# pouryashirazian/FemBrain

Hardware: AMD Instinct MI355X
Metric: FEM steps/sec (assemble+PCG) at 1M tets (higher is better)
Workload: dtype f64 arithmetic / f32 stored matrix

## Files before the change

fembrain_amd/csrc/fem_handle.h:

```cpp
#pragma once
#include "comm.h"
#include "common.h"
#include "fem_kernels.h"
#include "fem_plan.h"
#include "plan_device.h"
#include "renumber.h"
#include "delta.h"
#include "subdivide.h"
#include "surface.h"

namespace fb {

struct PipeKernel;

struct PersistState {
  int pipe_mir_knob = -1;
  int persist_fallbacks = 0;
  int persist_launches = 0;
  int persist_rearms = 0;
  double persist_seconds = 0;
  long long persist_iterations = 0;

  int pipe_lines_nodes = 0;
  double pipe_gather_lines[2] = {0, 0};

  bool persist = false;
  int persist_blocks = 0, persist_waves = 0;
  const PipeKernel* kernel = nullptr;
  int pipe_rows = 1;
  int pipe_wmax = 0;
  int pipe_slots_dealt = 0;
// ... 202 lines not shown
```

fembrain_amd/csrc/fem_persist.hip:

```cpp
#include <cmath>
#include <cstring>

#include "fem_handle.h"
#include "pcg_pipe.hip.h"
#include "pcg_pipe2.hip.h"
#include "pcg_pipe_plan.h"

using namespace fb;

namespace fb {

struct PipeKernel {
  int rows;
  bool c16;
  int wmax, klt;
  bool timing, shard, bj, help, xyz;
  const void* fn;
};

namespace {

#define FB_PIPE1(C16, WMAX, KLT, TIMING, SHARD, BJ, HELP, XYZ) \
  {1, C16, WMAX, KLT, TIMING, SHARD, BJ, HELP, XYZ, (const void*)k_pcg_pipe<float, C16, WMAX, KLT, TIMING, SHARD, BJ, HELP, XYZ>}
#define FB_PIPE2(C16, SHARD, XYZ) {2, C16, 12, kPipe2Klt, false, SHARD, false, false, XYZ, (const void*)k_pcg_pipe2<C16, SHARD, XYZ>}
// ... 32 lines not shown
  k.rearm = std::max(0, env_int("FEMBRAIN_PERSIST_REARM", 32));
  k.timing = getenv("FEMBRAIN_PERSIST_TIMING") ? std::max(1, env_int("FEMBRAIN_PERSIST_TIMING", 1)) : 0;
  k.poll_all = env_int("FEMBRAIN_PERSIST_POLL_ALL", 0) != 0;
  k.sharded = env_int("FEMBRAIN_SHARDED_PERSIST", 0) != 0;
  k.shard_relief = env_int("FEMBRAIN_SHARD_RELIEF", -1);
  k.balance = env_int("FEMBRAIN_PIPE_BALANCE", -1);
  k.small = env_int("FEMBRAIN_PIPE_SMALL", 0) != 0;
  k.klt7 = env_int("FEMBRAIN_PIPE_KLT7", 1) != 0;
  k.helpers = env_int("FEMBRAIN_PIPE_HELPERS", -1);
  k.help_minlen = env_int("FEMBRAIN_PIPE_HELP_MINLEN", 16);
  k.xyz = env_int("FEMBRAIN_PIPE_XYZ", -1);
  k.lds_by_width = env_int("FEMBRAIN_PIPE_LDS_BY_WIDTH", 0) != 0;
  k.lds_cap = getenv("FEMBRAIN_PIPE_LDS_CAP") ? std::max(1, env_int("FEMBRAIN_PIPE_LDS_CAP", 1)) : 0;
  k.plain_stores = env_int("FEMBRAIN_PIPE_PLAIN_STORES", -1);
  k.mirror = env_int("FEMBRAIN_PIPE_MIRROR", 1) != 0;
  k.verbose = getenv("FEMBRAIN_TIMING") != nullptr;
  return k;
}

int resolve_pipe_kernel(fb_fem_s* h, const PersistKnobs& kn) {
  PersistState& ps = h->ps;
  PipeKernel want;
  want.rows = ps.pipe_rows;
  want.shard = ps.shard_persist;
  want.bj = h->prm.pcg_variant == FB_PCG_BLOCK_JACOBI;
  want.help = ps.pipe_tasks.p != nullptr;
  want.xyz = ps.pipe_xyz;
  want.c16 = !want.shard && h->c16 != 0;
  want.timing = ps.persist_timing.p != nullptr && want.rows == 1;
  if (want.bj && want.timing) return fail(FB_EINVAL, "FEMBRAIN_PERSIST_TIMING is built for the Jacobi kernel");
// ... 204 lines not shown
  h->ps.sbox = nullptr;
  h->ps.shard_persist = false;
}

void read_persist_timeout(fb_fem_s* h) {
  const char* t = getenv("FEMBRAIN_PERSIST_TIMEOUT_MS");
  const double ms = t ? atof(t) : (h->plan.n_ranks > 1 ? 2000.0 : 50.0);
  h->ps.persist_timeout_ticks = std::max(1LL, (long long)(ms * 1e5));
}

int setup_persist(fb_fem_s* h) {
  const FemPlan& P = h->plan;
  PersistState& ps = h->ps;
  const PersistKnobs kn = read_persist_knobs();
  if (ps.pipe_mir_knob < 0) ps.pipe_mir_knob = kn.mirror ? 1 : 0;
  ps.pipe_timing_level = kn.timing;
  ps.reset_plan(kn.rearm);
  hipDeviceProp_t prop;
  FB_HIP(hipGetDeviceProperties(&prop, h->prm.device));
  const int nb = std::min(kPipeMaxBlocks, ((h->cu_limit > 0 ? std::min(h->cu_limit, prop.multiProcessorCount) : prop.multiProcessorCount) / 8) * 8);
  int w = nb >= 8 ? ceil_div(ceil_div(P.n_slices, 8), nb / 8) : 0;
  if (P.n_ranks == 1 && !P.slice_off.empty()) {
    w = pipe_deal_by_slots(P.slice_off.data(), P.n_slices, nb, w, kn, &ps.pipe_wg_first_host);
    if (!ps.pipe_wg_first_host.empty()) FB_TRY(ps.pipe_wg_first.upload(ps.pipe_wg_first_host, h->stream));
  }
  read_persist_timeout(h);
  const bool explicit_p = h->prm.pcg_variant == FB_PCG_PERSISTENT;
  const bool shard_opt = P.n_ranks > 1 && kn.sharded;
  if (explicit_p && P.n_ranks > 1 && !shard_opt) return fail(FB_EINVAL, "FB_PCG_PERSISTENT on a sharded handle needs FEMBRAIN_SHARDED_PERSIST=1 (unmeasured on multi-GPU hardware)");
  if (explicit_p && h->f64) return fail(FB_EINVAL, "FB_PCG_PERSISTENT needs FB_MATRIX_F32 storage (part of the matrix is kept in LDS as fp32 words)");
// ... 94 lines not shown
  const PipeKernel& K = *ps.kernel;
  PipeArgs pa;
  pa.post = ps.pipe_post.p; pa.flags = ps.pipe_flags.p; pa.error = ps.pipe_flags.p + ps.persist_blocks + ps.pipe_flag_extra + 4; pa.seqs = ps.pipe_flags.p + ps.persist_blocks + ps.pipe_flag_extra + 8;
  pa.producers = ps.pipe_prod.p; pa.prod_count = ps.pipe_prod_count.p; pa.prod_xcd = ps.pipe_prod_xcd.p; pa.plain_local = ps.pipe_plain_local; pa.xcc = ps.pipe_xcc.p;
  pa.start = start; pa.n_iters = n_iters; pa.eps2 = eps * eps; pa.max_iter = max_iter;
  pa.timeout_ticks = ps.persist_timeout_ticks;
  pa.timing = ps.persist_timing.p;
  pa.planes = ps.pipe_planes.p; pa.n_pad = ps.shard_persist ? (size_t)ceil_div(h->plan.n_local, 64) * 64 : (size_t)h->plan.n_slices * 64;
  pa.pstate = ps.pipe_state.p;
  pa.tasks = ps.pipe_tasks.p; pa.n_help = ps.pipe_n_help;
  pa.wg_first = ps.pipe_wg_first.p;
  pa.mirror = ps.pipe_mir.p; pa.mir_addr = ps.pipe_mir_addr.p; pa.mir_wg = ps.pipe_mir_wg.p; pa.mir_pool = ps.pipe_mir_pool.p;
  const int cwaves = K.rows == 2 ? ceil_div(ps.persist_waves, 2) : ps.persist_waves;
  pa.service = cwaves + ps.pipe_help_waves < ps.pipe_wmax ? 1 : 0;
  pa.prefetch_slots = ps.persist_waves >= 9 ? (K.rows == 2 ? 3 : 4) : 0;
  ShardArgs sa;
  memset(&sa, 0, sizeof sa);
  if (ps.shard_persist) {
    sa.rank = h->plan.rank; sa.n_ranks = h->plan.n_ranks; sa.n_owned = h->plan.n_owned; sa.n_halo = h->plan.n_local - h->plan.n_owned;
    sa.box = ps.sbox; sa.peer_box = ps.sbox_peers.p; sa.peer_seg = ps.sh_peer_seg.p; sa.halo_cap = ps.sbox_halo_cap;
    sa.halo_off = ps.sh_halo_off.p; sa.row_send_off = ps.sh_row_send_off.p; sa.row_send_rank = ps.sh_row_send_rank.p; sa.row_send_pos = ps.sh_row_send_pos.p;
    sa.wg_send_mask = ps.sh_wg_send_mask.p; sa.n_senders = ps.sh_n_senders.p; sa.proxy_wg = ps.sh_proxy_wg.p; sa.n_proxy = ps.sh_n_proxy; sa.wg_duty = ps.sh_wg_duty.p; sa.wg_range = ps.sh_wg_range.p;
    sa.delay_ticks = remote_delay_ticks();
  }
  SellView sv = sell_view(h);
  const float *vals = (const float*)h->vals.p, *dlo = (const float*)h->dlo.p;
  const double* inv = K.bj ? h->invblk.p : h->invdiag.p;
  void* args[] = {&sv, &vals, &dlo, &inv, &b, &h->x.p, &h->r.p, &h->Ad.p, &ps.pipe_z.p, &ps.pipe_s.p, &h->d.p, &h->st.p, &pa, &sa};
  const size_t lds = 160 * 1024;
  const dim3 grid(ps.persist_blocks), block(64 * (cwaves + ps.pipe_help_waves + pa.service));
// ... 192 lines not shown
```

fembrain_amd/csrc/pcg_pipe.hip.h:

```cpp
#pragma once
#include "fem_kernels.h"
#include "pcg_pipe_stream.hip.h"
#include "pcg_pipe_onchip.hip.h"
#include "pcg_pipe_mirror.h"

namespace fb {

constexpr int kPipeMaxWaves = 12;
constexpr int kPipeMaxBlocks = 256;
constexpr int kPipeSyncDoubles = 2 * 16 + 2 * kPipeMaxBlocks + 8;
constexpr int kPipeMaxProducers = 64;
constexpr int pipe_slot_bytes(bool c16) { return c16 ? 9 * 256 + 128 : 10 * 256; }
constexpr int pipe_lds_slots(bool c16) { return c16 ? 65 : 62; }
static_assert(sizeof(double) * kPipeSyncDoubles + (size_t)pipe_lds_slots(false) * pipe_slot_bytes(false) <= 160 * 1024, "LDS budget of k_pcg_pipe");
static_assert(sizeof(double) * kPipeSyncDoubles + (size_t)pipe_lds_slots(true) * pipe_slot_bytes(true) <= 160 * 1024, "LDS budget of k_pcg_pipe<c16>");
static_assert(mir_slot_bytes(true) == pipe_slot_bytes(true) && mir_slot_bytes(false) == pipe_slot_bytes(false) && mir_lds_slots(true) == pipe_lds_slots(true) &&
              mir_lds_slots(false) == pipe_lds_slots(false) && kMirWaves == kPipeMaxWaves, "the LDS window's planner sees the kernel's LDS");
static_assert(pipe_lds_slots(true) * pipe_slot_bytes(true) / 4 < 65536 && pipe_lds_slots(false) * pipe_slot_bytes(false) / 4 < 65536, "16-bit LDS word addresses of the mirror layers");

struct PipeArgs {
  unsigned long long* post;
  unsigned int* flags;
  unsigned int* error;
  unsigned int* seqs;
  const int* producers;
  const int* prod_count;
  const int* prod_xcd;
  int plain_local;
  unsigned int* xcc;
  int prefetch_slots;
  int service;
  int start;
  int n_iters;
  double eps2;
  int max_iter;
  long long timeout_ticks;
  long long* timing;
  double* planes;
  size_t n_pad;
  double* pstate;
  const int* wg_first;
  const int4* tasks;
  int n_help;
// ... 405 lines not shown
    if (rvalid) {
      if (XYZ && through) {
        st_sc1_xyz(pl + 3 * (size_t)row, vin[0], vin[1], vin[2]);
      } else if (through) {
#pragma unroll
        for (int a = 0; a < 3; a++) st_sc1_f64(pl + a * xs + cs * (size_t)row, vin[a]);
      } else {
#pragma unroll
        for (int a = 0; a < 3; a++) pl[a * xs + cs * (size_t)row] = vin[a];
      }
      if constexpr (SHARD) shard_send_row(sa, BL, pub, send_beg, send_end, vin);
    }
  };
  auto product = [&](const double* vin, double* y, bool post_sums, bool late_acquire) {
    double* pl = pa.planes + (size_t)(pub & 1u) * 3 * pa.n_pad;
    asm volatile("s_waitcnt vmcnt(0)" ::: "memory");
    __syncthreads();
    lap(0);
    if (post_sums) sums++;
    if (wv != 0 && live && pa.prefetch_slots > 0 && (mir_a > 0 || own_k1 > k_after)) {
      int so_k = so + (mir_a > 0 ? 0 : k_after);
      asm volatile("" : "+s"(so_k));
      pipe_prefetch_values(min(pa.prefetch_slots, mir_a > 0 ? mir_a : own_k1 - k_after), ((unsigned int)so_k * 9u * 64u + (unsigned int)lane) * (unsigned int)sizeof(float), vals);
    }
    if constexpr (SHARD) {
      if (spare) shard_service_product(sa, BL, pa, pub, pl, nb, lane, send_mask, t_limit, bc, failed);
    }
    if (wv == 0) {
      if (lane == 0) st_sc1_u32(pa.flags + blockIdx.x, pub);
      if (post_sums && lane < 2) {
        double t = 0.0;
        for (int w = 0; w < n_waves; w++) t += wsum[lane * 16 + w];
        const unsigned long long bits = (unsigned long long)__double_as_longlong(t), tag = (unsigned long long)sums << 32;
        unsigned long long* post = pa.post + ((size_t)(sums & 1u) * nb + blockIdx.x) * 4 + 2 * lane;
        st_sc1_u64(post, (bits >> 32) | tag);
// ... 27 lines not shown
      }
      if (failed && lane == 0) st_sc1_u32(pa.error, 1u);
      if (late_acquire) __builtin_amdgcn_fence(__ATOMIC_ACQUIRE, "agent");
      if (plain_cand && !xcc_known && !failed) {
        const bool same = my_prod < 0 || ld_sc1_u32(pa.xcc + my_prod) == ((pub << 4) | my_xcc);
        const bool all_same = __ballot(!same) == 0ULL;
        if (lane == 0) bc[5] = all_same ? 1.0 : 0.0;
      }
      asm volatile("s_waitcnt vmcnt(0)" ::: "memory");
      if (lane == 0) bc[3] = (failed || ld_sc1_u32(pa.error) != 0u) ? 1.0 : 0.0;
    }
    __syncthreads();
    lap(1);
    if (uniform_flag(bc[3] != 0.0 || (SHARD && bc[4] != 0.0))) { failed = true; return; }
    if (plain_cand && !xcc_known) { through = !uniform_flag(bc[5] != 0.0); xcc_known = true; }
    double y0 = 0, y1 = 0, y2 = 0;
    if (rvalid) {
      MT u00 = m00, u01 = m01, u02 = m02, u11 = m11, u12 = m12, u22 = m22;
      asm volatile("" : "+v"(u00), "+v"(u01), "+v"(u02), "+v"(u11), "+v"(u12), "+v"(u22));
      const double l00 = (double)u00, l01 = (double)u01, l02 = (double)u02, l11 = (double)u11, l12 = (double)u12, l22 = (double)u22;
      y0 = l00 * vin[0] + l01 * vin[1] + l02 * vin[2];
      y1 = l01 * vin[0] + l11 * vin[1] + l12 * vin[2];
      y2 = l02 * vin[0] + l12 * vin[1] + l22 * vin[2];
    }
    long long tseam = tprev;
    if (live) {
      if constexpr (kMir) {
        if (mir_a > 0) {
          int so_k = so;
          asm volatile("" : "+s"(so_k));
          pipe_stream_slots<C16, XYZ>(mir_a, ((unsigned int)so_k * 9u * 64u + (unsigned int)lane) * (unsigned int)sizeof(float),
                                      ((unsigned int)so_k * 64u + (unsigned int)lane) * (unsigned int)(C16 ? sizeof(short) : sizeof(int)), vals,
                                      C16 ? (const void*)sv.coldelta : (const void*)sv.colidx, pl, pl + xs, pl + 2 * xs, row, y0, y1, y2);
        }
        seam(5, tseam);
        const char* lbase = (const char*)(lds + kPipeSyncDoubles);
        pipe_onchip_slots<C16>(mir_m, max(KL, 0), (const unsigned int*)(lbase + mir_tab) + lane, (const unsigned short*)(lbase + mir_tab) + lane, lres, lcd, lbase, pl, pl + xs,
                               pl + 2 * xs, row, y0, y1, y2);
      }
      if (sizeof(MT) == 4 && KLT >= 16) {
        double gx[KLT][3];
#pragma unroll
        for (int k = 0; k < KLT; k++) {
          const unsigned int col = k < KL ? lds_col(k) : 0u;
          const double* xp = pl + cs * (size_t)col;
          gx[k][0] = k < KL ? xp[0] : 0.0; gx[k][1] = k < KL ? xp[xs] : 0.0; gx[k][2] = k < KL ? xp[2 * xs] : 0.0;
        }
#pragma unroll
        for (int k = 0; k < KLT; k++) if (k < KL) {
          const unsigned int* lk = lres + (size_t)k * kValWords * 64;
          const double x0 = gx[k][0], x1 = gx[k][1], x2 = gx[k][2];
          y0 += (double)__uint_as_float(lk[0 * 64]) * x0 + (double)__uint_as_float(lk[1 * 64]) * x1 + (double)__uint_as_float(lk[2 * 64]) * x2;
          y1 += (double)__uint_as_float(lk[3 * 64]) * x0 + (double)__uint_as_float(lk[4 * 64]) * x1 + (double)__uint_as_float(lk[5 * 64]) * x2;
// ... 288 lines not shown
```

fembrain_amd/csrc/pcg_pipe_plan.h:

```cpp
#pragma once
#include <algorithm>
#include <cstdio>
#include <cstdlib>
#include <vector>

#include "common.h"
#include "fem_plan.h"
#include "pcg_pipe2.hip.h"

namespace fb {

struct PersistKnobs {
  int pcg_persist = -1;
  int min_waves = 2;
  bool rows2 = false;
  int rearm = 32;
  int timing = 0;
  bool poll_all = false;
  bool sharded = false;
  int shard_relief = -1;
  int balance = -1;
  bool small = false;
  bool klt7 = true;
  int helpers = -1;
  int help_minlen = 16;
  int xyz = -1;
  bool lds_by_width = false;
  int lds_cap = 0;
  int plain_stores = -1;
  bool mirror = true;
  bool verbose = false;
};

inline int pipe_deal_by_slots(const int* slice_off, int n_slices, int nb, int w, const PersistKnobs& kn, std::vector<int>* wg_first) {
  wg_first->clear();
  if (nb < 8 || w < 1 || w > 2 * kPipeMaxWaves) return w;
  const int per = nb / 8, chunk = ceil_div(n_slices, 8), cap = w <= kPipeMaxWaves ? kPipeMaxWaves : 2 * kPipeMaxWaves;
  long long total = 0, worst = 0;
  for (int b = 0; b < nb; b++) {
    int first, count;
    pipe_slices(n_slices, nb, b, &first, &count);
    const long long sl = count > 0 ? slice_off[first + count] - slice_off[first] : 0;
    total += sl;
    worst = std::max(worst, sl);
  }
// ... 232 lines not shown
```

fembrain_amd/csrc/pcg_pipe_stream.hip.h:

```cpp
#pragma once
#include <hip/hip_runtime.h>

namespace fb {

#define FBP_LOADV(r0, r1, r2, r3, r4, r5, r6, r7, r8)                      \
  "global_load_dword " r0 ", %[voff], %[svals]\n\t"                        \
  "global_load_dword " r1 ", %[voff], %[svals] offset:256\n\t"             \
  "global_load_dword " r2 ", %[voff], %[svals] offset:512\n\t"             \
  "global_load_dword " r3 ", %[voff], %[svals] offset:768\n\t"             \
  "global_load_dword " r4 ", %[voff], %[svals] offset:1024\n\t"            \
  "global_load_dword " r5 ", %[voff], %[svals] offset:1280\n\t"            \
  "global_load_dword " r6 ", %[voff], %[svals] offset:1536\n\t"            \
  "global_load_dword " r7 ", %[voff], %[svals] offset:1792\n\t"            \
  "global_load_dword " r8 ", %[voff], %[svals] offset:2048\n\t"            \
  "v_add_u32_e32 %[voff], 0x900, %[voff]\n\t"
#define FBP_LOADV_A FBP_LOADV("v136", "v137", "v138", "v139", "v140", "v141", "v142", "v143", "v144")
#define FBP_LOADV_B FBP_LOADV("v145", "v146", "v147", "v148", "v149", "v150", "v151", "v152", "v153")
#define FBP_LOADC16(c) "global_load_sshort " c ", %[coff], %[scols]\n\t" "v_add_u32_e32 %[coff], 0x80, %[coff]\n\t"
#define FBP_LOADC32(c) "global_load_dword " c ", %[coff], %[scols]\n\t" "v_add_u32_e32 %[coff], 0x100, %[coff]\n\t"
#define FBP_GOFF16(c) "v_add_u32_e32 v122, %[row], " c "\n\t" "v_lshlrev_b32_e32 v122, 3, v122\n\t"
#define FBP_GOFF32(c) "v_lshlrev_b32_e32 v122, 3, " c "\n\t"
#define FBP_GOFF16X(c) "v_add_u32_e32 v122, %[row], " c "\n\t" "v_mul_u32_u24_e32 v122, 24, v122\n\t"
#define FBP_GOFF32X(c) "v_mul_u32_u24_e32 v122, 24, " c "\n\t"
#define FBP_GATHER(g0, g1, g2)                                             \
// ... 22 lines not shown
  FBP_ROW("%[y1]", "v139", "v140", "v141", "v[124:125]", "v[126:127]", "v[128:129]")           \
  FBP_ROW("%[y2]", "v142", "v143", "v144", "v[124:125]", "v[126:127]", "v[128:129]")
#define FBP_COMPUTE_B                                                                          \
  FBP_ROW("%[y0]", "v145", "v146", "v147", "v[130:131]", "v[132:133]", "v[134:135]")           \
  FBP_ROW("%[y1]", "v148", "v149", "v150", "v[130:131]", "v[132:133]", "v[134:135]")           \
  FBP_ROW("%[y2]", "v151", "v152", "v153", "v[130:131]", "v[132:133]", "v[134:135]")
#define FBP_FULL(LOADC, GOFF, cX, cY, LOADV_Y, GATHER_Y, COMPUTE_X, W1, W2) \
  LOADC(cX) LOADV_Y "s_waitcnt vmcnt(" W1 ")\n\t" GOFF(cY) GATHER_Y "s_waitcnt vmcnt(" W2 ")\n\t" COMPUTE_X
#define FBP_PENULT(GOFF, cY, LOADV_Y, GATHER_Y, COMPUTE_X, W3, W4)         \
  LOADV_Y "s_waitcnt vmcnt(" W3 ")\n\t" GOFF(cY) GATHER_Y "s_waitcnt vmcnt(" W4 ")\n\t" COMPUTE_X
#define FBP_LAST(COMPUTE_X) "s_waitcnt vmcnt(0)\n\t" COMPUTE_X
#define FBP_BODY(LOADC, GOFF) FBP_BODYG(LOADC, GOFF, FBP_GATHER_A, FBP_GATHER_B, "22", "13", "21", "12")
#define FBP_BODYG(LOADC, GOFF, GATHER_A, GATHER_B, W1, W2, W3, W4)                                                                                 \
           \
  "s_nop 4\n\t"                                                                                                 \
                         \
  LOADC("v154")                                                                                                 \
  "s_cmp_lt_i32 %[n], 2\n\t"                                                                                    \
  "s_cbranch_scc1 .Lfbp_one_%=\n\t"                                                                             \
  LOADC("v155")                                                                                                 \
  FBP_LOADV_A                                                                                                   \
  "s_waitcnt vmcnt(10)\n\t"                                                                                     \
  "s_branch .Lfbp_g0_%=\n"                                                                                      \
  ".Lfbp_one_%=:\n\t"                                                                                           \
  FBP_LOADV_A                                                                                                   \
  "s_waitcnt vmcnt(9)\n"                                                                                        \
  ".Lfbp_g0_%=:\n\t"                                                                                            \
  GOFF("v154") GATHER_A                                                                                     \
                                                                                 \
  ".Lfbp_even_%=:\n\t"                                                                                          \
  "s_cmp_lt_i32 %[n], 3\n\t"                                                                                    \
  "s_cbranch_scc1 .Lfbp_even_tail_%=\n\t"                                                                       \
  FBP_FULL(LOADC, GOFF, "v154", "v155", FBP_LOADV_B, GATHER_B, FBP_COMPUTE_A, W1, W2)                               \
  "s_sub_i32 %[n], %[n], 1\n\t"                                                                                 \
                                                                                  \
  "s_cmp_lt_i32 %[n], 3\n\t"                                                                                    \
  "s_cbranch_scc1 .Lfbp_odd_tail_%=\n\t"                                                                        \
  FBP_FULL(LOADC, GOFF, "v155", "v154", FBP_LOADV_A, GATHER_A, FBP_COMPUTE_B, W1, W2)                               \
  "s_sub_i32 %[n], %[n], 1\n\t"                                                                                 \
  "s_branch .Lfbp_even_%=\n"                                                                                    \
  ".Lfbp_even_tail_%=:\n\t"                                                                                     \
  "s_cmp_lt_i32 %[n], 2\n\t"                                                                                    \
  "s_cbranch_scc1 .Lfbp_even_last_%=\n\t"                                                                       \
  FBP_PENULT(GOFF, "v155", FBP_LOADV_B, GATHER_B, FBP_COMPUTE_A, W3, W4)                                            \
  FBP_LAST(FBP_COMPUTE_B)                                                                                       \
  "s_branch .Lfbp_end_%=\n"                                                                                     \
  ".Lfbp_even_last_%=:\n\t"                                                                                     \
  FBP_LAST(FBP_COMPUTE_A)                                                                                       \
  "s_branch .Lfbp_end_%=\n"                                                                                     \
  ".Lfbp_odd_tail_%=:\n\t"                                                                                      \
  "s_cmp_lt_i32 %[n], 2\n\t"                                                                                    \
  "s_cbranch_scc1 .Lfbp_odd_last_%=\n\t"                                                                        \
  FBP_PENULT(GOFF, "v154", FBP_LOADV_A, GATHER_A, FBP_COMPUTE_B, W3, W4)                                            \
  FBP_LAST(FBP_COMPUTE_A)                                                                                       \
  "s_branch .Lfbp_end_%=\n"                                                                                     \
  ".Lfbp_odd_last_%=:\n\t"                                                                                      \
  FBP_LAST(FBP_COMPUTE_B)                                                                                       \
  ".Lfbp_end_%=:\n\t"
#define FBP_CLOBBERS                                                                                                                   \
  "memory", "scc", "v120", "v121", "v122", "v123", "v124", "v125", "v126", "v127", "v128", "v129", "v130", "v131", "v132", "v133",      \
  "v134", "v135", "v136", "v137", "v138", "v139", "v140", "v141", "v142", "v143", "v144", "v145", "v146", "v147", "v148", "v149",      \
  "v150", "v151", "v152", "v153", "v154", "v155"

__device__ __forceinline__ void pipe_prefetch_values(int n, unsigned int voff, const float* vals);

template <typename T>
__device__ __forceinline__ T* scalar_ptr(T* p) {
  const unsigned long long b = (unsigned long long)p;
  const unsigned int lo = __builtin_amdgcn_readfirstlane((unsigned int)b), hi = __builtin_amdgcn_readfirstlane((unsigned int)(b >> 32));
  return (T*)(((unsigned long long)hi << 32) | lo);
}

__device__ __forceinline__ void pipe_prefetch_values(int n, unsigned int voff, const float* vals) {
  vals = scalar_ptr(vals);
  n = __builtin_amdgcn_readfirstlane(n);
  asm volatile("s_nop 4\n\t"
               "s_cmp_lt_i32 %[n], 1\n\t"
// ... 32 lines not shown
                 : [svals] "s"(vals), [scols] "s"(cols), [spl0] "s"(pl0), [spl1] "s"(pl1), [spl2] "s"(pl2), [row] "v"(row)
                 : FBP_CLOBBERS);
  } else if (C16) {
    asm volatile(FBP_BODY(FBP_LOADC16, FBP_GOFF16)
                 : [y0] "+v"(y0), [y1] "+v"(y1), [y2] "+v"(y2), [voff] "+v"(voff), [coff] "+v"(coff), [n] "+s"(n)
                 : [svals] "s"(vals), [scols] "s"(cols), [spl0] "s"(pl0), [spl1] "s"(pl1), [spl2] "s"(pl2), [row] "v"(row)
                 : FBP_CLOBBERS);
  } else {
    asm volatile(FBP_BODY(FBP_LOADC32, FBP_GOFF32)
                 : [y0] "+v"(y0), [y1] "+v"(y1), [y2] "+v"(y2), [voff] "+v"(voff), [coff] "+v"(coff), [n] "+s"(n)
                 : [svals] "s"(vals), [scols] "s"(cols), [spl0] "s"(pl0), [spl1] "s"(pl1), [spl2] "s"(pl2), [row] "v"(row)
                 : FBP_CLOBBERS);
  }
}

}
```

fembrain_amd/csrc/plan_api.cpp:

```cpp
#include <cstring>
#include <string>
#include <vector>

#include "../../include/fembrain_hip.h"
#include "../../include/fembrain_hip_testing.h"
#include "fem_plan.h"
#include "renumber.h"
#include "pcg_pipe_mirror.h"

namespace fb {
int fail(int code, const char* fmt, ...);
}

struct fb_plan_s {
  fb::FemPlan plan;
};

extern "C" {

int fb_plan_create(fb_plan_t* out, int n_nodes, int n_tets, const int* tets, int n_fixed_dofs, const int* fixed_dofs, int n_ranks,
                   int rank, const int* node_splits) {
  if (!out) return fb::fail(FB_EINVAL, "null output");
  fb_plan_s* p = new fb_plan_s;
  int rc = fb::build_fem_plan(p->plan, n_nodes, n_tets, tets, n_fixed_dofs, fixed_dofs, n_ranks, rank, node_splits);
  if (rc != FB_OK) {
    delete p;
    return rc;
  }
  *out = p;
  return FB_OK;
}
// ... 48 lines not shown
  if (rc != FB_OK) return rc;
  memcpy(old_of_new, o.data(), sizeof(int) * (size_t)n_nodes);
  return FB_OK;
}

int fb_plan_shard_vote(int n_nodes, int n_tets, const int* tets, int n_ranks, int rank, const int* node_splits, int out[3]) {
  if (!tets || !out) return fb::fail(FB_EINVAL, "null argument");
  unsigned long long sum = 0;
  int splits_sum = 0;
  fb::shard_neighbour_count(n_nodes, n_tets, tets, n_ranks, rank, node_splits, &out[0], &sum, &splits_sum, &out[1], &out[2]);
  return FB_OK;
}

int fb_plan_mirror_model(fb_plan_t p, int nb, int c16, int klt, int out[4]) {
  if (!p || !out || nb < 8 || (nb & 7) || (klt != 6 && klt != 7)) return fb::fail(FB_EINVAL, "bad argument");
  const fb::FemPlan& P = p->plan;
  const int* so = P.slice_off.data();
  const int* ci = P.colidx.data();
  out[0] = out[1] = out[3] = 0;
  out[2] = 1 << 30;
  for (int b = 0; b < nb; b++) {
    const int xcd = b & 7, j = b >> 3, per = nb >> 3, chunk = (P.n_slices + 7) >> 3, lo_s = xcd * chunk;
    int len = P.n_slices - lo_s;
    len = len < 0 ? 0 : (len > chunk ? chunk : len);
    const int base = len / per, rem = len - base * per;
    const int first = lo_s + j * base + (j < rem ? j : rem);
    const int count = std::min(base + (j < rem ? 1 : 0), fb::kMirWaves);
    if (count <= 0) continue;
    const int lo = first * 64, hi = std::min((first + count) * 64, P.n_owned);
    fb::MirWave mw[fb::kMirWaves];
    for (int w = 0; w < count; w++) {
      const int sl = first + w, width = so[sl + 1] - so[sl];
      int hist[256] = {0};
      for (int l = 0; l < 64; l++) {
        const int dk = fb::mir_lane_diag(so, ci, sl, l, P.n_owned);
        if (dk >= 0 && dk < 256) hist[dk]++;
      }
      int d = -1, best = 0;
      for (int k = 0; k < width && k < 256; k++)
        if (hist[k] > best) { best = hist[k]; d = k; }
      int m = 0;
      if (d >= 0)
        for (; m < fb::kMirMax && d - 1 - m >= 0; m++) {
          int n = 0;
          for (int l = 0; l < 64; l++) n += fb::mir_lane_lower(so, ci, sl, d - 1 - m, l, lo, hi) ? 1 : 0;
          if (n < fb::kMirLanes) break;
        }
      mw[w].d = d; mw[w].m = m; mw[w].width = width;
    }
    auto misses = [&]() {
      int e = 0;
      for (int w = 0; w < count; w++)
        for (int k = 0; k < mw[w].m; k++)
          for (int l = 0; l < 64; l++) e += fb::mir_lane_addr(so, ci, first, mw, w, k, l, lo, hi, c16 != 0) < 0 ? 1 : 0;
      return e;
    };
    bool ok = fb::mir_wg_layout(mw, count, klt, c16 != 0, 0, false);
    int E = ok ? misses() : 0;
    ok = ok && E <= fb::kMirPoolMax && fb::mir_wg_layout(mw, count, klt, c16 != 0, E, true);
    if (ok) { E = misses(); ok = fb::mir_wg_gains(mw, count, klt, c16 != 0); }
    if (!ok) { fb::mir_wg_plain(mw, count, klt, c16 != 0); E = 0; }
    for (int w = 0; w < count; w++) { out[0] += mw[w].m; out[2] = std::min(out[2], mw[w].p); }
    out[1] += E;
    out[3] += ok ? 1 : 0;
  }
  return FB_OK;
}

}
```

fembrain_amd/lib.py:

```python
import ctypes as C
import os
import subprocess

import numpy as np

_HERE = os.path.dirname(os.path.abspath(__file__))
LIB_PATH = os.path.join(_HERE, "libfembrain_hip.so")

FB_OK, FB_EINVAL, FB_EDEVICE, FB_ENOMEM, FB_ESOLVER, FB_ECOMM = 0, -1, -2, -3, -4, -5
FB_MATRIX_F32, FB_MATRIX_F64, FB_MATRIX_AUTO = 0, 1, 2
FB_XCH_COLLECTIVE, FB_XCH_P2P, FB_XCH_P2P_SUMS, FB_XCH_P2P_FUSED = 1, 2, 3, 4
FB_PCG_MERGED, FB_PCG_REFERENCE, FB_PCG_PERSISTENT, FB_PCG_BLOCK_JACOBI = 0, 1, 3, 4
FB_PCG_PATH_TWO_LAUNCH, FB_PCG_PATH_PERSISTENT, FB_PCG_PATH_FALLBACK, FB_PCG_PATH_RESOLVED = 0, 1, 2, 3
FB_SPMV_AUTO, FB_SPMV_ROWS, FB_SPMV_SPLIT = 0, 1, 2
FB_INTEGRATOR_VOLUME_CONSERVING, FB_INTEGRATOR_NEWMARK = 0, 1
FB_RENUMBER_AUTO, FB_RENUMBER_ON, FB_RENUMBER_OFF = 0, 1, -1
FB_RESYNC_FULL, FB_RESYNC_DELTA_MERGED, FB_RESYNC_DELTA_REBUILT = 0, 1, 2
FB_CUT_BAKE, FB_CUT_CARRY = 0, 1
FB_CUT_NOTHING, FB_CUT_DONE, FB_CUT_UNHANDLED, FB_CUT_DRY = 0, 1, 2, 3
FB_CUT_UNHANDLED_IDS = 64

_dp = C.POINTER(C.c_double)
_fp = C.POINTER(C.c_float)
_ip = C.POINTER(C.c_int)
# ... 137 lines not shown
        "fb_comm_info": (C.c_int, [vp, _ip, _ip, _ip]),
        "fb_comm_create_local": (C.c_int, [C.POINTER(vp), C.c_int, C.c_int, C.c_char_p, C.c_size_t, C.c_int]),
        "fb_comm_test_allgather": (C.c_int, [vp, C.c_void_p, C.c_void_p, C.c_size_t]),
        "fb_fem_create_from_poly": (C.c_int, [C.POINTER(vp), vp, C.c_int, _ip, C.POINTER(FemParams)]),
        "fb_fem_device_plan_get": (C.c_longlong, [vp, C.c_char_p, _ip, C.c_longlong]),
        "fb_fem_plan_on_device": (C.c_int, [vp]),
        "fb_fem_assembly_kernel": (C.c_int, [vp]),
        "fb_fem_assembly_wide_slices": (C.c_int, [vp]),
        "fb_plan_create": (C.c_int, [C.POINTER(vp), C.c_int, C.c_int, _ip, C.c_int, _ip, C.c_int, C.c_int, _ip]),
        "fb_plan_destroy": (C.c_int, [vp]),
        "fb_plan_slab_order": (C.c_int, [C.c_int, _dp, C.c_int, _ip, _ip, _ip, _ip]),
        "fb_plan_shard_vote": (C.c_int, [C.c_int, C.c_int, _ip, C.c_int, C.c_int, _ip, _ip]),
        "fb_plan_info": (C.c_int, [vp, _ip]),
        "fb_plan_get": (C.c_int, [vp, C.c_char_p, _ip, C.c_size_t]),
        "fb_plan_mirror_model": (C.c_int, [vp, C.c_int, C.c_int, C.c_int, _ip]),
    }
    poly_sig = {
        "fb_fem_transport": (C.c_int, [vp]),
        "fb_fem_set_exchange_mode": (C.c_int, [vp, C.c_int]),
        "fb_fem_persist_rearms": (C.c_int, [vp]),
        "fb_fem_persist_helpers": (C.c_int, [vp]),
        "fb_fem_persist_gather": (C.c_int, [vp, C.POINTER(C.c_double), C.POINTER(C.c_double)]),
        "fb_fem_persist_mirror": (C.c_int, [vp, _ip, _ip, _ip]),
        "fb_fem_renumbering": (C.c_int, [vp, _ip, _ip]),
        "fb_fem_owned_nodes": (C.c_int, [vp, _ip]),
        "fb_fem_halo_info": (C.c_int, [vp, _ip, _ip]),
        "fb_fem_sharded_persist": (C.c_int, [vp]),
        "fb_fem_set_sharded_persist": (C.c_int, [vp, C.c_int]),
        "fb_fem_time_exchange": (C.c_int, [vp, C.c_int, _dp, _dp]),
        "fb_fem_time_element_stiffness": (C.c_int, [vp, C.c_int, _dp]),
# ... 84 lines not shown
```

include/fembrain_hip_testing.h:

```cpp
#ifndef FEMBRAIN_HIP_TESTING_H
#define FEMBRAIN_HIP_TESTING_H
#include <stddef.h>
#ifdef __cplusplus
extern "C" {
#endif

typedef struct fb_plan_s* fb_plan_t;

int fb_plan_create(fb_plan_t* out, int n_nodes, int n_tets, const int* tets, int n_fixed_dofs, const int* fixed_dofs,
                   int n_ranks, int rank, const int* node_splits);
int fb_plan_destroy(fb_plan_t p);
int fb_plan_info(fb_plan_t p, int info[12]);
int fb_plan_get(fb_plan_t p, const char* name, int* out, size_t capacity);

int fb_plan_mirror_model(fb_plan_t p, int nb, int c16, int klt, int out[4]);

int fb_plan_slab_order(int n_nodes, const double* xyz, int n_tets, const int* tets, int* old_of_new, int* span_caller, int* span_internal);

int fb_plan_shard_vote(int n_nodes, int n_tets, const int* tets, int n_ranks, int rank, const int* node_splits, int out[3]);

struct fb_comm_s;
int fb_comm_create_local(struct fb_comm_s** out, int rank, int n_ranks, const char* shm_name, size_t outbox_bytes, int device);
int fb_comm_test_allgather(struct fb_comm_s* c, const void* mine, void* all, size_t bytes);

int fb_poly_compile_info(int n_ops, const float* ops16, int n_prims, const float* prims20, int* n_steps, int* n_slots);

#ifdef __cplusplus
}
#endif
#endif
```

Before: 67.74.

## Add opt-in held-slot preload for mirrored PCG pipe SpMV streaming

Adds a FEMBRAIN_PIPE_HOLD knob, off by default, that preloads the first one or two mirrored matrix slots into registers before the barrier. The streamed SpMV then starts from those held values instead of reloading them. It also moves the diagonal-block product ahead of the barrier, passes the on-chip slot pointers differently, and factors the mirror model into a helper exposed through a new window-model query. The goal is to hide global-memory latency at the start of each product, at the cost of more vector registers and more complex inline assembly.

Measured after the change: 66.45. 0.981x the previous value.

```diff
diff --git a/fembrain_amd/csrc/fem_handle.h b/fembrain_amd/csrc/fem_handle.h
--- a/fembrain_amd/csrc/fem_handle.h
+++ b/fembrain_amd/csrc/fem_handle.h
@@ -15,6 +15,7 @@
 
 struct PersistState {
   int pipe_mir_knob = -1;
+  int pipe_hold_knob = -1;
   int persist_fallbacks = 0;
   int persist_launches = 0;
   int persist_rearms = 0;
diff --git a/fembrain_amd/csrc/fem_persist.hip b/fembrain_amd/csrc/fem_persist.hip
--- a/fembrain_amd/csrc/fem_persist.hip
+++ b/fembrain_amd/csrc/fem_persist.hip
@@ -70,6 +70,7 @@
   k.lds_cap = getenv("FEMBRAIN_PIPE_LDS_CAP") ? std::max(1, env_int("FEMBRAIN_PIPE_LDS_CAP", 1)) : 0;
   k.plain_stores = env_int("FEMBRAIN_PIPE_PLAIN_STORES", -1);
   k.mirror = env_int("FEMBRAIN_PIPE_MIRROR", 1) != 0;
+  k.hold = env_int("FEMBRAIN_PIPE_HOLD", 0) != 0;
   k.verbose = getenv("FEMBRAIN_TIMING") != nullptr;
   return k;
 }
@@ -304,6 +305,7 @@
   PersistState& ps = h->ps;
   const PersistKnobs kn = read_persist_knobs();
   if (ps.pipe_mir_knob < 0) ps.pipe_mir_knob = kn.mirror ? 1 : 0;
+  if (ps.pipe_hold_knob < 0) ps.pipe_hold_knob = kn.hold ? 1 : 0;
   ps.pipe_timing_level = kn.timing;
   ps.reset_plan(kn.rearm);
   hipDeviceProp_t prop;
@@ -428,6 +430,7 @@
   const int cwaves = K.rows == 2 ? ceil_div(ps.persist_waves, 2) : ps.persist_waves;
   pa.service = cwaves + ps.pipe_help_waves < ps.pipe_wmax ? 1 : 0;
   pa.prefetch_slots = ps.persist_waves >= 9 ? (K.rows == 2 ? 3 : 4) : 0;
+  pa.hold = ps.pipe_hold_knob != 0 ? 1 : 0;
   ShardArgs sa;
   memset(&sa, 0, sizeof sa);
   if (ps.shard_persist) {
diff --git a/fembrain_amd/csrc/pcg_pipe.hip.h b/fembrain_amd/csrc/pcg_pipe.hip.h
--- a/fembrain_amd/csrc/pcg_pipe.hip.h
+++ b/fembrain_amd/csrc/pcg_pipe.hip.h
@@ -27,6 +27,7 @@
   const int* prod_count;
   const int* prod_xcd;
   int plain_local;
+  int hold;
   unsigned int* xcc;
   int prefetch_slots;
   int service;
@@ -462,11 +463,33 @@
   };
   auto product = [&](const double* vin, double* y, bool post_sums, bool late_acquire) {
     double* pl = pa.planes + (size_t)(pub & 1u) * 3 * pa.n_pad;
+    double y0 = 0, y1 = 0, y2 = 0;
+    auto diag_low = [&]() {
+      if (rvalid) {
+        MT u00 = m00, u01 = m01, u02 = m02, u11 = m11, u12 = m12, u22 = m22;
+        asm volatile("" : "+v"(u00), "+v"(u01), "+v"(u02), "+v"(u11), "+v"(u12), "+v"(u22));
+        const double l00 = (double)u00, l01 = (double)u01, l02 = (double)u02, l11 = (double)u11, l12 = (double)u12, l22 = (double)u22;
+        y0 = l00 * vin[0] + l01 * vin[1] + l02 * vin[2];
+        y1 = l01 * vin[0] + l11 * vin[1] + l12 * vin[2];
+        y2 = l02 * vin[0] + l12 * vin[1] + l22 * vin[2];
+      }
+    };
+    if constexpr (kMir) diag_low();
     asm volatile("s_waitcnt vmcnt(0)" ::: "memory");
     __syncthreads();
     lap(0);
     if (post_sums) sums++;
-    if (wv != 0 && live && pa.prefetch_slots > 0 && (mir_a > 0 || own_k1 > k_after)) {
+    PipeHeld hs;
+    int held = 0;
+    if constexpr (kMir) {
+      held = __builtin_amdgcn_readfirstlane(wv != 0 && live && pa.hold != 0 ? min(mir_a, 2) : 0);
+      int so_k = so;
+      asm volatile("" : "+s"(so_k));
+      pipe_hold_preload<C16>(held, min(pa.prefetch_slots, mir_a) - held, ((unsigned int)so_k * 9u * 64u + (unsigned int)lane) * (unsigned int)sizeof(float),
+                             ((unsigned int)so_k * 64u + (unsigned int)lane) * (unsigned int)(C16 ? sizeof(short) : sizeof(int)), vals,
+                             C16 ? (const void*)sv.coldelta : (const void*)sv.colidx, hs);
+    }
+    if (wv != 0 && live && held == 0 && pa.prefetch_slots > 0 && (mir_a > 0 || own_k1 > k_after)) {
       int so_k = so + (mir_a > 0 ? 0 : k_after);
       asm volatile("" : "+s"(so_k));
       pipe_prefetch_values(min(pa.prefetch_slots, mir_a > 0 ? mir_a : own_k1 - k_after), ((unsigned int)so_k * 9u * 64u + (unsigned int)lane) * (unsigned int)sizeof(float), vals);
@@ -524,29 +547,23 @@
     lap(1);
     if (uniform_flag(bc[3] != 0.0 || (SHARD && bc[4] != 0.0))) { failed = true; return; }
     if (plain_cand && !xcc_known) { through = !uniform_flag(bc[5] != 0.0); xcc_known = true; }
-    double y0 = 0, y1 = 0, y2 = 0;
-    if (rvalid) {
-      MT u00 = m00, u01 = m01, u02 = m02, u11 = m11, u12 = m12, u22 = m22;
-      asm volatile("" : "+v"(u00), "+v"(u01), "+v"(u02), "+v"(u11), "+v"(u12), "+v"(u22));
-      const double l00 = (double)u00, l01 = (double)u01, l02 = (double)u02, l11 = (double)u11, l12 = (double)u12, l22 = (double)u22;
-      y0 = l00 * vin[0] + l01 * vin[1] + l02 * vin[2];
-      y1 = l01 * vin[0] + l11 * vin[1] + l12 * vin[2];
-      y2 = l02 * vin[0] + l12 * vin[1] + l22 * vin[2];
-    }
+    if constexpr (!kMir) diag_low();
     long long tseam = tprev;
     if (live) {
       if constexpr (kMir) {
         if (mir_a > 0) {
-          int so_k = so;
+          int so_k = so + held;
           asm volatile("" : "+s"(so_k));
-          pipe_stream_slots<C16, XYZ>(mir_a, ((unsigned int)so_k * 9u * 64u + (unsigned int)lane) * (unsigned int)sizeof(float),
-                                      ((unsigned int)so_k * 64u + (unsigned int)lane) * (unsigned int)(C16 ? sizeof(short) : sizeof(int)), vals,
-                                      C16 ? (const void*)sv.coldelta : (const void*)sv.colidx, pl, pl + xs, pl + 2 * xs, row, y0, y1, y2);
+          pipe_stream_held<C16>(mir_a, held, ((unsigned int)so_k * 9u * 64u + (unsigned int)lane) * (unsigned int)sizeof(float),
+                                ((unsigned int)so_k * 64u + (unsigned int)lane) * (unsigned int)(C16 ? sizeof(short) : sizeof(int)), vals,
+                                C16 ? (const void*)sv.coldelta : (const void*)sv.colidx, pl, pl + xs, pl + 2 * xs, row, hs, y0, y1, y2);
         }
         seam(5, tseam);
         const char* lbase = (const char*)(lds + kPipeSyncDoubles);
-        pipe_onchip_slots<C16>(mir_m, max(KL, 0), (const unsigned int*)(lbase + mir_tab) + lane, (const unsigned short*)(lbase + mir_tab) + lane, lres, lcd, lbase, pl, pl + xs,
-                               pl + 2 * xs, row, y0, y1, y2);
+        int lane_o = lane;
+        asm volatile("" : "+v"(lane_o));
+        pipe_onchip_slots<C16>(mir_m, max(KL, 0), (const unsigned int*)(lbase + mir_tab) + lane_o, (const unsigned short*)(lbase + mir_tab) + lane_o,
+                               (const unsigned int*)lwave + lane_o, (const short*)(lwave + (size_t)klt_w * 9 * 256) + lane_o, lbase, pl, pl + xs, pl + 2 * xs, row, y0, y1, y2);
       }
       if (sizeof(MT) == 4 && KLT >= 16) {
         double gx[KLT][3];
diff --git a/fembrain_amd/csrc/pcg_pipe_plan.h b/fembrain_amd/csrc/pcg_pipe_plan.h
--- a/fembrain_amd/csrc/pcg_pipe_plan.h
+++ b/fembrain_amd/csrc/pcg_pipe_plan.h
@@ -29,6 +29,7 @@
   int lds_cap = 0;
   int plain_stores = -1;
   bool mirror = true;
+  bool hold = false;
   bool verbose = false;
 };
 
diff --git a/fembrain_amd/csrc/pcg_pipe_stream.hip.h b/fembrain_amd/csrc/pcg_pipe_stream.hip.h
--- a/fembrain_amd/csrc/pcg_pipe_stream.hip.h
+++ b/fembrain_amd/csrc/pcg_pipe_stream.hip.h
@@ -60,53 +60,112 @@
 #define FBP_BODYG(LOADC, GOFF, GATHER_A, GATHER_B, W1, W2, W3, W4)                                                                                 \
            \
   "s_nop 4\n\t"                                                                                                 \
-                         \
-  LOADC("v154")                                                                                                 \
+  FBP_PROLOGUE(LOADC, GOFF, "v154", "v155", FBP_LOADV_A, GATHER_A)                                              \
+  FBP_STEADY(LOADC, GOFF, "v154", "v155", FBP_LOADV_A, FBP_LOADV_B, GATHER_A, GATHER_B, FBP_COMPUTE_A, FBP_COMPUTE_B, W1, W2, W3, W4)
+#define FBP_PROLOGUE(LOADC, GOFF, cA, cB, LOADV_A, GATHER_A)                                                    \
+  LOADC(cA)                                                                                                     \
   "s_cmp_lt_i32 %[n], 2\n\t"                                                                                    \
   "s_cbranch_scc1 .Lfbp_one_%=\n\t"                                                                             \
-  LOADC("v155")                                                                                                 \
-  FBP_LOADV_A                                                                                                   \
+  LOADC(cB)                                                                                                     \
+  LOADV_A                                                                                                       \
   "s_waitcnt vmcnt(10)\n\t"                                                                                     \
   "s_branch .Lfbp_g0_%=\n"                                                                                      \
   ".Lfbp_one_%=:\n\t"                                                                                           \
-  FBP_LOADV_A                                                                                                   \
+  LOADV_A                                                                                                       \
   "s_waitcnt vmcnt(9)\n"                                                                                        \
   ".Lfbp_g0_%=:\n\t"                                                                                            \
-  GOFF("v154") GATHER_A                                                                                     \
+  GOFF(cA) GATHER_A
+#define FBP_STEADY(LOADC, GOFF, cA, cB, LOADV_A, LOADV_B, GATHER_A, GATHER_B, COMPUTE_A, COMPUTE_B, W1, W2, W3, W4) \
                                                                                  \
   ".Lfbp_even_%=:\n\t"                                                                                          \
   "s_cmp_lt_i32 %[n], 3\n\t"                                                                                    \
   "s_cbranch_scc1 .Lfbp_even_tail_%=\n\t"                                                                       \
-  FBP_FULL(LOADC, GOFF, "v154", "v155", FBP_LOADV_B, GATHER_B, FBP_COMPUTE_A, W1, W2)                               \
+  FBP_FULL(LOADC, GOFF, cA, cB, LOADV_B, GATHER_B, COMPUTE_A, W1, W2)                                           \
   "s_sub_i32 %[n], %[n], 1\n\t"                                                                                 \
                                                                                   \
   "s_cmp_lt_i32 %[n], 3\n\t"                                                                                    \
   "s_cbranch_scc1 .Lfbp_odd_tail_%=\n\t"                                                                        \
-  FBP_FULL(LOADC, GOFF, "v155", "v154", FBP_LOADV_A, GATHER_A, FBP_COMPUTE_B, W1, W2)                               \
+  FBP_FULL(LOADC, GOFF, cB, cA, LOADV_A, GATHER_A, COMPUTE_B, W1, W2)                                           \
   "s_sub_i32 %[n], %[n], 1\n\t"                                                                                 \
   "s_branch .Lfbp_even_%=\n"                                                                                    \
   ".Lfbp_even_tail_%=:\n\t"                                                                                     \
   "s_cmp_lt_i32 %[n], 2\n\t"                                                                                    \
   "s_cbranch_scc1 .Lfbp_even_last_%=\n\t"                                                                       \
-  FBP_PENULT(GOFF, "v155", FBP_LOADV_B, GATHER_B, FBP_COMPUTE_A, W3, W4)                                            \
-  FBP_LAST(FBP_COMPUTE_B)                                                                                       \
+  FBP_PENULT(GOFF, cB, LOADV_B, GATHER_B, COMPUTE_A, W3, W4)                                                    \
+  FBP_LAST(COMPUTE_B)                                                                                           \
   "s_branch .Lfbp_end_%=\n"                                                                                     \
   ".Lfbp_even_last_%=:\n\t"                                                                                     \
-  FBP_LAST(FBP_COMPUTE_A)                                                                                       \
+  FBP_LAST(COMPUTE_A)                                                                                           \
   "s_branch .Lfbp_end_%=\n"                                                                                     \
   ".Lfbp_odd_tail_%=:\n\t"                                                                                      \
   "s_cmp_lt_i32 %[n], 2\n\t"                                                                                    \
   "s_cbranch_scc1 .Lfbp_odd_last_%=\n\t"                                                                        \
-  FBP_PENULT(GOFF, "v154", FBP_LOADV_A, GATHER_A, FBP_COMPUTE_B, W3, W4)                                            \
-  FBP_LAST(FBP_COMPUTE_A)                                                                                       \
+  FBP_PENULT(GOFF, cA, LOADV_A, GATHER_A, COMPUTE_B, W3, W4)                                                    \
+  FBP_LAST(COMPUTE_A)                                                                                           \
   "s_branch .Lfbp_end_%=\n"                                                                                     \
   ".Lfbp_odd_last_%=:\n\t"                                                                                      \
-  FBP_LAST(FBP_COMPUTE_B)                                                                                       \
+  FBP_LAST(COMPUTE_B)                                                                                           \
   ".Lfbp_end_%=:\n\t"
+#define FBP_HV_A "%[a0]", "%[a1]", "%[a2]", "%[a3]", "%[a4]", "%[a5]", "%[a6]", "%[a7]", "%[a8]"
+#define FBP_HV_B "%[b0]", "%[b1]", "%[b2]", "%[b3]", "%[b4]", "%[b5]", "%[b6]", "%[b7]", "%[b8]"
+#define FBP_EXPAND(M, ...) M(__VA_ARGS__)
+#define FBP_LOADV_HA FBP_EXPAND(FBP_LOADV, FBP_HV_A)
+#define FBP_LOADV_HB FBP_EXPAND(FBP_LOADV, FBP_HV_B)
+#define FBP_COMPUTE_HA                                                                         \
+  FBP_ROW("%[y0]", "%[a0]", "%[a1]", "%[a2]", "v[124:125]", "v[126:127]", "v[128:129]")        \
+  FBP_ROW("%[y1]", "%[a3]", "%[a4]", "%[a5]", "v[124:125]", "v[126:127]", "v[128:129]")        \
+  FBP_ROW("%[y2]", "%[a6]", "%[a7]", "%[a8]", "v[124:125]", "v[126:127]", "v[128:129]")
+#define FBP_COMPUTE_HB                                                                         \
+  FBP_ROW("%[y0]", "%[b0]", "%[b1]", "%[b2]", "v[130:131]", "v[132:133]", "v[134:135]")        \
+  FBP_ROW("%[y1]", "%[b3]", "%[b4]", "%[b5]", "v[130:131]", "v[132:133]", "v[134:135]")        \
+  FBP_ROW("%[y2]", "%[b6]", "%[b7]", "%[b8]", "v[130:131]", "v[132:133]", "v[134:135]")
+#define FBP_BODYH(LOADC, GOFF)                                                                                  \
+  "s_nop 4\n\t"                                                                                                 \
+  "s_cmp_lt_i32 %[held], 1\n\t"                                                                                 \
+  "s_cbranch_scc1 .Lfbp_h0_%=\n\t"                                                                              \
+  GOFF("%[ca]") FBP_GATHER_A                                                                                    \
+  "s_cmp_lt_i32 %[held], 2\n\t"                                                                                 \
+  "s_cbranch_scc1 .Lfbp_even_last_%=\n\t"                                         \
+  GOFF("%[cb]") FBP_GATHER_B                                                                                    \
+  "s_cmp_lt_i32 %[n], 3\n\t"                                                                                    \
+  "s_cbranch_scc1 .Lfbp_hw3_%=\n\t"                                                                             \
+  LOADC("%[ca]")                                                                                                \
+  "s_cmp_lt_i32 %[n], 4\n\t"                                                                                    \
+  "s_cbranch_scc1 .Lfbp_hw4_%=\n\t"                                                                             \
+  LOADC("%[cb]")                                                                                                \
+  "s_waitcnt vmcnt(5)\n\t"                                   \
+  "s_branch .Lfbp_hc0_%=\n"                                                                                     \
+  ".Lfbp_hw4_%=:\n\t"                                                                                           \
+  "s_waitcnt vmcnt(4)\n\t"                                                                                      \
+  "s_branch .Lfbp_hc0_%=\n"                                                                                     \
+  ".Lfbp_hw3_%=:\n\t"                                                                                           \
+  "s_waitcnt vmcnt(3)\n"                                                                                        \
+  ".Lfbp_hc0_%=:\n\t"                                                                                           \
+  FBP_COMPUTE_HA                                                                                                \
+  "s_cmp_lt_i32 %[n], 3\n\t"                                                                                    \
+  "s_cbranch_scc1 .Lfbp_odd_last_%=\n\t"                                \
+  FBP_LOADV_HA                                                                                                  \
+  "s_cmp_lt_i32 %[n], 4\n\t"                                                                                    \
+  "s_cbranch_scc1 .Lfbp_hw9_%=\n\t"                                                                             \
+  "s_waitcnt vmcnt(10)\n\t"                               \
+  "s_branch .Lfbp_hg2_%=\n"                                                                                     \
+  ".Lfbp_hw9_%=:\n\t"                                                                                           \
+  "s_waitcnt vmcnt(9)\n"                                                                                        \
+  ".Lfbp_hg2_%=:\n\t"                                                                                           \
+  GOFF("%[ca]") FBP_GATHER_A                                                                                    \
+  FBP_COMPUTE_HB                                                                                                \
+  "s_sub_i32 %[n], %[n], 2\n\t"                                                                                 \
+  "s_branch .Lfbp_even_%=\n"                                                                                    \
+  ".Lfbp_h0_%=:\n\t"                                                                                            \
+  FBP_PROLOGUE(LOADC, GOFF, "%[ca]", "%[cb]", FBP_LOADV_HA, FBP_GATHER_A)                                       \
+  FBP_STEADY(LOADC, GOFF, "%[ca]", "%[cb]", FBP_LOADV_HA, FBP_LOADV_HB, FBP_GATHER_A, FBP_GATHER_B, FBP_COMPUTE_HA, FBP_COMPUTE_HB, "22", "13", "21", "12")
 #define FBP_CLOBBERS                                                                                                                   \
   "memory", "scc", "v120", "v121", "v122", "v123", "v124", "v125", "v126", "v127", "v128", "v129", "v130", "v131", "v132", "v133",      \
   "v134", "v135", "v136", "v137", "v138", "v139", "v140", "v141", "v142", "v143", "v144", "v145", "v146", "v147", "v148", "v149",      \
   "v150", "v151", "v152", "v153", "v154", "v155"
+#define FBP_CLOBBERS_HELD                                                                                                              \
+  "memory", "scc", "v120", "v121", "v122", "v123", "v124", "v125", "v126", "v127", "v128", "v129", "v130", "v131", "v132", "v133",      \
+  "v134", "v135"
 
 __device__ __forceinline__ void pipe_prefetch_values(int n, unsigned int voff, const float* vals);
 
@@ -169,4 +228,59 @@
   }
 }
 
-}
+struct PipeHeld {
+  float a[9], b[9];
+  int ca, cb;
+};
+
+template <bool C16>
+__device__ __forceinline__ void pipe_hold_preload(int held, int more, unsigned int voff, unsigned int coff, const float* vals, const void* cols, PipeHeld& h) {
+  vals = scalar_ptr(vals); cols = scalar_ptr(cols);
+  held = __builtin_amdgcn_readfirstlane(held); more = __builtin_amdgcn_readfirstlane(more);
+#define FBP_PRELOAD(LOADC)                                                                                                     \
+  asm volatile("s_nop 4\n\t"                                                                                                   \
+               "s_cmp_lt_i32 %[held], 1\n\t"                                                                                   \
+               "s_cbranch_scc1 .Lfbp_hp_end_%=\n\t"                                                                            \
+               LOADC("%[ca]") FBP_LOADV_HA                                                                                     \
+               "s_cmp_lt_i32 %[held], 2\n\t"                                                                                   \
+               "s_cbranch_scc1 .Lfbp_hp_wait_%=\n\t"   \
+               LOADC("%[cb]") FBP_LOADV_HB                                                                                     \
+               "s_cmp_lt_i32 %[more], 1\n\t"                                                                                   \
+               "s_cbranch_scc1 .Lfbp_hp_wait_%=\n\t"                                                                           \
+               FBP_LOADV("v120", "v121", "v122", "v123", "v124", "v125", "v126", "v127", "v128")                               \
+               "s_cmp_lt_i32 %[more], 2\n\t"                                                                                   \
+               "s_cbranch_scc1 .Lfbp_hp_wait_%=\n\t"                                                                           \
+               FBP_LOADV("v120", "v121", "v122", "v123", "v124", "v125", "v126", "v127", "v128")                               \
+               ".Lfbp_hp_wait_%=:\n\t"                                                                                         \
+               "s_waitcnt vmcnt(0)\n"                                                                                          \
+               ".Lfbp_hp_end_%=:\n\t"                                                                                          \
+               : [a0] "=&v"(h.a[0]), [a1] "=&v"(h.a[1]), [a2] "=&v"(h.a[2]), [a3] "=&v"(h.a[3]), [a4] "=&v"(h.a[4]), [a5] "=&v"(h.a[5]),     \
+                 [a6] "=&v"(h.a[6]), [a7] "=&v"(h.a[7]), [a8] "=&v"(h.a[8]), [b0] "=&v"(h.b[0]), [b1] "=&v"(h.b[1]), [b2] "=&v"(h.b[2]),     \
+                 [b3] "=&v"(h.b[3]), [b4] "=&v"(h.b[4]), [b5] "=&v"(h.b[5]), [b6] "=&v"(h.b[6]), [b7] "=&v"(h.b[7]), [b8] "=&v"(h.b[8]),     \
+                 [ca] "=&v"(h.ca), [cb] "=&v"(h.cb), [voff] "+v"(voff), [coff] "+v"(coff)                                        \
+               : [held] "s"(held), [more] "s"(more), [svals] "s"(vals), [scols] "s"(cols)                                     \
+               : FBP_CLOBBERS_HELD)
+  if (C16) FBP_PRELOAD(FBP_LOADC16);
+  else FBP_PRELOAD(FBP_LOADC32);
+#undef FBP_PRELOAD
+}
+
+template <bool C16>
+__device__ __forceinline__ void pipe_stream_held(int n, int held, unsigned int voff, unsigned int coff, const float* vals, const void* cols, const double* pl0,
+                                                 const double* pl1, const double* pl2, int row, PipeHeld& h, double& y0, double& y1, double& y2) {
+  vals = scalar_ptr(vals); cols = scalar_ptr(cols); pl0 = scalar_ptr(pl0); pl1 = scalar_ptr(pl1); pl2 = scalar_ptr(pl2);
+  n = __builtin_amdgcn_readfirstlane(n); held = __builtin_amdgcn_readfirstlane(held);
+#define FBP_HELD_OPERANDS                                                                                                      \
+               : [y0] "+v"(y0), [y1] "+v"(y1), [y2] "+v"(y2), [voff] "+v"(voff), [coff] "+v"(coff), [n] "+s"(n),               \
+                 [a0] "+v"(h.a[0]), [a1] "+v"(h.a[1]), [a2] "+v"(h.a[2]), [a3] "+v"(h.a[3]), [a4] "+v"(h.a[4]), [a5] "+v"(h.a[5]),     \
+                 [a6] "+v"(h.a[6]), [a7] "+v"(h.a[7]), [a8] "+v"(h.a[8]), [b0] "+v"(h.b[0]), [b1] "+v"(h.b[1]), [b2] "+v"(h.b[2]),     \
+                 [b3] "+v"(h.b[3]), [b4] "+v"(h.b[4]), [b5] "+v"(h.b[5]), [b6] "+v"(h.b[6]), [b7] "+v"(h.b[7]), [b8] "+v"(h.b[8]),     \
+                 [ca] "+v"(h.ca), [cb] "+v"(h.cb)                                                                              \
+               : [held] "s"(held), [svals] "s"(vals), [scols] "s"(cols), [spl0] "s"(pl0), [spl1] "s"(pl1), [spl2] "s"(pl2), [row] "v"(row) \
+               : FBP_CLOBBERS_HELD
+  if (C16) asm volatile(FBP_BODYH(FBP_LOADC16, FBP_GOFF16) FBP_HELD_OPERANDS);
+  else asm volatile(FBP_BODYH(FBP_LOADC32, FBP_GOFF32) FBP_HELD_OPERANDS);
+#undef FBP_HELD_OPERANDS
+}
+
+}
diff --git a/fembrain_amd/csrc/plan_api.cpp b/fembrain_amd/csrc/plan_api.cpp
--- a/fembrain_amd/csrc/plan_api.cpp
+++ b/fembrain_amd/csrc/plan_api.cpp
@@ -15,6 +15,53 @@
 struct fb_plan_s {
   fb::FemPlan plan;
 };
+
+static int mirror_model_wg(const fb::FemPlan& P, int nb, int b, bool c16, int klt, fb::MirWave* mw, int* pool, bool* mirrors) {
+  const int* so = P.slice_off.data();
+  const int* ci = P.colidx.data();
+  const int xcd = b & 7, j = b >> 3, per = nb >> 3, chunk = (P.n_slices + 7) >> 3, lo_s = xcd * chunk;
+  int len = P.n_slices - lo_s;
+  len = len < 0 ? 0 : (len > chunk ? chunk : len);
+  const int base = len / per, rem = len - base * per;
+  const int first = lo_s + j * base + (j < rem ? j : rem);
+  const int count = std::min(base + (j < rem ? 1 : 0), fb::kMirWaves);
+  *pool = 0; *mirrors = false;
+  if (count <= 0) return 0;
+  const int lo = first * 64, hi = std::min((first + count) * 64, P.n_owned);
+  for (int w = 0; w < count; w++) {
+    const int sl = first + w, width = so[sl + 1] - so[sl];
+    int hist[256] = {0};
+    for (int l = 0; l < 64; l++) {
+      const int dk = fb::mir_lane_diag(so, ci, sl, l, P.n_owned);
+      if (dk >= 0 && dk < 256) hist[dk]++;
+    }
+    int d = -1, best = 0;
+    for (int k = 0; k < width && k < 256; k++)
+      if (hist[k] > best) { best = hist[k]; d = k; }
+    int m = 0;
+    if (d >= 0)
+      for (; m < fb::kMirMax && d - 1 - m >= 0; m++) {
+        int n = 0;
+        for (int l = 0; l < 64; l++) n += fb::mir_lane_lower(so, ci, sl, d - 1 - m, l, lo, hi) ? 1 : 0;
+        if (n < fb::kMirLanes) break;
+      }
+    mw[w].d = d; mw[w].m = m; mw[w].width = width;
+  }
+  auto misses = [&]() {
+    int e = 0;
+    for (int w = 0; w < count; w++)
+      for (int k = 0; k < mw[w].m; k++)
+        for (int l = 0; l < 64; l++) e += fb::mir_lane_addr(so, ci, first, mw, w, k, l, lo, hi, c16) < 0 ? 1 : 0;
+    return e;
+  };
+  bool ok = fb::mir_wg_layout(mw, count, klt, c16, 0, false);
+  int E = ok ? misses() : 0;
+  ok = ok && E <= fb::kMirPoolMax && fb::mir_wg_layout(mw, count, klt, c16, E, true);
+  if (ok) { E = misses(); ok = fb::mir_wg_gains(mw, count, klt, c16); }
+  if (!ok) { fb::mir_wg_plain(mw, count, klt, c16); E = 0; }
+  *pool = E; *mirrors = ok;
+  return count;
+}
 
 extern "C" {
 
@@ -93,52 +140,14 @@
 
 int fb_plan_mirror_model(fb_plan_t p, int nb, int c16, int klt, int out[4]) {
   if (!p || !out || nb < 8 || (nb & 7) || (klt != 6 && klt != 7)) return fb::fail(FB_EINVAL, "bad argument");
-  const fb::FemPlan& P = p->plan;
-  const int* so = P.slice_off.data();
-  const int* ci = P.colidx.data();
   out[0] = out[1] = out[3] = 0;
   out[2] = 1 << 30;
   for (int b = 0; b < nb; b++) {
-    const int xcd = b & 7, j = b >> 3, per = nb >> 3, chunk = (P.n_slices + 7) >> 3, lo_s = xcd * chunk;
-    int len = P.n_slices - lo_s;
-    len = len < 0 ? 0 : (len > chunk ? chunk : len);
-    const int base = len / per, rem = len - base * per;
-    const int first = lo_s + j * base + (j < rem ? j : rem);
-    const int count = std::min(base + (j < rem ? 1 : 0), fb::kMirWaves);
+    fb::MirWave mw[fb::kMirWaves];
+    int E = 0;
+    bool ok = false;
+    const int count = mirror_model_wg(p->plan, nb, b, c16 != 0, klt, mw, &E, &ok);
     if (count <= 0) continue;
-    const int lo = first * 64, hi = std::min((first + count) * 64, P.n_owned);
-    fb::MirWave mw[fb::kMirWaves];
-    for (int w = 0; w < count; w++) {
-      const int sl = first + w, width = so[sl + 1] - so[sl];
-      int hist[256] = {0};
-      for (int l = 0; l < 64; l++) {
-        const int dk = fb::mir_lane_diag(so, ci, sl, l, P.n_owned);
-        if (dk >= 0 && dk < 256) hist[dk]++;
-      }
-      int d = -1, best = 0;
-      for (int k = 0; k < width && k < 256; k++)
-        if (hist[k] > best) { best = hist[k]; d = k; }
-      int m = 0;
-      if (d >= 0)
-        for (; m < fb::kMirMax && d - 1 - m >= 0; m++) {
-          int n = 0;
-          for (int l = 0; l < 64; l++) n += fb::mir_lane_lower(so, ci, sl, d - 1 - m, l, lo, hi) ? 1 : 0;
-          if (n < fb::kMirLanes) break;
-        }
-      mw[w].d = d; mw[w].m = m; mw[w].width = width;
-    }
-    auto misses = [&]() {
-      int e = 0;
-      for (int w = 0; w < count; w++)
-        for (int k = 0; k < mw[w].m; k++)
-          for (int l = 0; l < 64; l++) e += fb::mir_lane_addr(so, ci, first, mw, w, k, l, lo, hi, c16 != 0) < 0 ? 1 : 0;
-      return e;
-    };
-    bool ok = fb::mir_wg_layout(mw, count, klt, c16 != 0, 0, false);
-    int E = ok ? misses() : 0;
-    ok = ok && E <= fb::kMirPoolMax && fb::mir_wg_layout(mw, count, klt, c16 != 0, E, true);
-    if (ok) { E = misses(); ok = fb::mir_wg_gains(mw, count, klt, c16 != 0); }
-    if (!ok) { fb::mir_wg_plain(mw, count, klt, c16 != 0); E = 0; }
     for (int w = 0; w < count; w++) { out[0] += mw[w].m; out[2] = std::min(out[2], mw[w].p); }
     out[1] += E;
     out[3] += ok ? 1 : 0;
@@ -146,4 +155,21 @@
   return FB_OK;
 }
 
+int fb_plan_window_model(fb_plan_t p, int nb, int c16, int klt, int* out, size_t capacity) {
+  if (!p || nb < 8 || (nb & 7) || (klt != 6 && klt != 7)) return fb::fail(FB_EINVAL, "bad argument");
+  size_t n = 0;
+  for (int b = 0; b < nb; b++) {
+    fb::MirWave mw[fb::kMirWaves];
+    int E = 0;
+    bool ok = false;
+    const int count = mirror_model_wg(p->plan, nb, b, c16 != 0, klt, mw, &E, &ok);
+    for (int w = 0; w < count; w++, n++)
+      if (out) {
+        if (3 * (n + 1) > capacity) return fb::fail(FB_EINVAL, "capacity %zu too small", capacity);
+        out[3 * n] = mw[w].a; out[3 * n + 1] = mw[w].m; out[3 * n + 2] = mw[w].p;
+      }
+  }
+  return (int)n;
 }
+
+}
diff --git a/fembrain_amd/lib.py b/fembrain_amd/lib.py
--- a/fembrain_amd/lib.py
+++ b/fembrain_amd/lib.py
@@ -175,6 +175,7 @@
         "fb_plan_info": (C.c_int, [vp, _ip]),
         "fb_plan_get": (C.c_int, [vp, C.c_char_p, _ip, C.c_size_t]),
         "fb_plan_mirror_model": (C.c_int, [vp, C.c_int, C.c_int, C.c_int, _ip]),
+        "fb_plan_window_model": (C.c_int, [vp, C.c_int, C.c_int, C.c_int, _ip, C.c_size_t]),
     }
     poly_sig = {
         "fb_fem_transport": (C.c_int, [vp]),
diff --git a/include/fembrain_hip_testing.h b/include/fembrain_hip_testing.h
--- a/include/fembrain_hip_testing.h
+++ b/include/fembrain_hip_testing.h
@@ -15,6 +15,8 @@
 
 int fb_plan_mirror_model(fb_plan_t p, int nb, int c16, int klt, int out[4]);
 
+int fb_plan_window_model(fb_plan_t p, int nb, int c16, int klt, int* out, size_t capacity);
+
 int fb_plan_slab_order(int n_nodes, const double* xyz, int n_tets, const int* tets, int* old_of_new, int* span_caller, int* span_internal);
 
 int fb_plan_shard_vote(int n_nodes, int n_tets, const int* tets, int n_ranks, int rank, const int* node_splits, int out[3]);
```
